# afiaka87/clip-guided-diffusion

Hardware: AMD Instinct MI355X
Metric: diffusion steps/sec (UNet+CLIP+grad) at 256x256 cutn=16 (higher is better)
Workload: dtype bf16x3 (split-bf16 MFMA, fp32 accumulate, fp32 storage); 1 GPU; BASELINE configs[1]: 256x256 class-cond UNet (554M), respace 250, cutn 16, batch 1/GPU, CLIP ViT-B/32, cgs 1000 tv 150 range 50, randomize_class, p_sample; global_batch=1, world_size_checked=1, collectives=none (single process)

## Files before the change

### clip-guided-diffusion_amd/csrc/vit.hip

```cpp
#include <memory>

#include "../../include/cgd_mi355x.h"
#include "net.h"

void ClipBlock::add_params(NetBase& net, const std::string& prefix, int width, int nheads) {
  pre = prefix;
  W = width;
  heads = nheads;
  net.add_param(pre + ".ln_1.weight", W);
  net.add_param(pre + ".ln_1.bias", W);
  net.add_param(pre + ".attn.in_proj_weight", (int64_t)3 * W * W);
  net.add_param(pre + ".attn.in_proj_bias", 3 * W);
  net.add_param(pre + ".attn.out_proj.weight", (int64_t)W * W);
  net.add_param(pre + ".attn.out_proj.bias", W);
  net.add_param(pre + ".ln_2.weight", W);
  net.add_param(pre + ".ln_2.bias", W);
  net.add_param(pre + ".mlp.c_fc.weight", (int64_t)4 * W * W);
  net.add_param(pre + ".mlp.c_fc.bias", 4 * W);
  net.add_param(pre + ".mlp.c_proj.weight", (int64_t)4 * W * W);
  net.add_param(pre + ".mlp.c_proj.bias", W);
}

void ClipBlock::lookup(NetBase& net) {
  ln1g = net.P(pre + ".ln_1.weight"); ln1b = net.P(pre + ".ln_1.bias");
  inw = net.P(pre + ".attn.in_proj_weight"); inb = net.P(pre + ".attn.in_proj_bias");
  ow = net.P(pre + ".attn.out_proj.weight"); ob = net.P(pre + ".attn.out_proj.bias");
  ln2g = net.P(pre + ".ln_2.weight"); ln2b = net.P(pre + ".ln_2.bias");
  fcw = net.P(pre + ".mlp.c_fc.weight"); fcb = net.P(pre + ".mlp.c_fc.bias");
  pjw = net.P(pre + ".mlp.c_proj.weight"); pjb = net.P(pre + ".mlp.c_proj.bias");
}

int clip_block_fwd(NetBase& net, const ClipBlock& b, ClipActs& t, const float* x, float* xo, int N, int T, bool causal, hipStream_t s) {
  cgd_ctx* ctx = net.ctx;
  const int W = b.W;
  const long rows = (long)N * T;
  CGD_TRY(net.ensure(t.st1, rows * 2)); CGD_TRY(net.ensure(t.st2, rows * 2));
  CGD_TRY(net.ensure(t.y, rows * W)); CGD_TRY(net.ensure(t.qkv, rows * 3 * W)); CGD_TRY(net.ensure(t.a, rows * W));
  CGD_TRY(net.ensure(t.x1, rows * W)); CGD_TRY(net.ensure(t.y2, rows * W)); CGD_TRY(net.ensure(t.u, rows * 4 * W));
  CGD_TRY(net.ensure(t.ga, rows * 4 * W));
  CGD_TRY(cgd_launch_ln_fwd(ctx, x, W, t.y.p, W, (int)rows, W, b.ln1g, b.ln1b, 1e-5f, t.st1.p, s));
  CGD_TRY(cgd_launch_gemm(ctx, lin(t.y.p, W, b.inw, W, t.qkv.p, 3 * W, b.inb, nullptr, 0, rows, 3 * W), s));
  const AttnShape sh{N, b.heads, T, W / b.heads, W, 0, causal ? 1 : 0};
  CGD_TRY(net.attn_fwd(t.att, sh, t.qkv.p, 3 * W, t.a.p, W, s));
  CGD_TRY(cgd_launch_gemm(ctx, lin(t.a.p, W, b.ow, W, t.x1.p, W, b.ob, x, W, rows, W, 1), s));
  CGD_TRY(cgd_launch_ln_fwd(ctx, t.x1.p, W, t.y2.p, W, (int)rows, W, b.ln2g, b.ln2b, 1e-5f, t.st2.p, s));
  {
    GemmParams fc = lin(t.y2.p, W, b.fcw, W, t.u.p, 4 * W, b.fcb, nullptr, 0, rows, 4 * W);
    if (cgd_gemm_fuses_act(ctx, fc)) {
      fc.act_out = t.ga.p; fc.ld_act = 4 * W; fc.act = b.act;
      CGD_TRY(cgd_launch_gemm(ctx, fc, s));
    } else {
      CGD_TRY(cgd_launch_gemm(ctx, fc, s));
      CGD_TRY(cgd_launch_act_fwd(ctx, t.u.p, t.ga.p, rows * 4 * W, b.act, s));
    }
  }
  return cgd_launch_gemm(ctx, lin(t.ga.p, 4 * W, b.pjw, 4 * W, xo, W, b.pjb, t.x1.p, W, rows, W, 1), s);
}

namespace {

struct Layer : ClipBlock {
  float *inwT = 0, *owT = 0, *fcwT = 0, *pjwT = 0;
  ClipActs f;
  DevBuf xo;
  DevBuf dga, du, dy2, dx1, da, dqkv, dy, dx;
};

struct ViT : NetBase {
  cgd_vit_config cfg;
  int g = 0, L = 0, W = 0, PP = 0;
  std::vector<Layer> layers;
  float *convw = 0, *convwT = 0, *cls = 0, *pos = 0, *lnpre_g = 0, *lnpre_b = 0, *lnpost_g = 0, *lnpost_b = 0, *proj = 0, *projT = 0;
  int N = 0, layout = 0;
  bool have_fwd = false;
  int fwd_prec = 0;
  DevBuf cols, pe, tok, st_pre, x0, st_post, clsn, dclsn, dxl, dtok, dcols;

  int build();
  int finalize(hipStream_t s);
  int forward(const float* img, int layout, int N, float* emb, hipStream_t s);
  int dgrad(const float* demb, float* dimg, hipStream_t s);
};

int ViT::build() {
  g = cfg.resolution / cfg.patch;
  L = g * g + 1;
  W = cfg.width;
  PP = 3 * cfg.patch * cfg.patch;
  if (cfg.resolution % cfg.patch) CGD_FAIL(ctx, "vit: resolution must be a multiple of the patch size");
  if (W % cfg.heads || (W / cfg.heads) % 4) CGD_FAIL(ctx, "vit: bad head configuration");
  add_param("conv1.weight", (int64_t)W * PP);
  add_param("class_embedding", W);
  add_param("positional_embedding", (int64_t)L * W);
  add_param("ln_pre.weight", W);
  add_param("ln_pre.bias", W);
  layers.resize(cfg.layers);
  for (int l = 0; l < cfg.layers; ++l) layers[l].add_params(*this, "transformer.resblocks." + std::to_string(l), W, cfg.heads);
  add_param("ln_post.weight", W);
  add_param("ln_post.bias", W);
  add_param("proj", (int64_t)W * cfg.out_dim);
  return 0;
}

int ViT::finalize(hipStream_t s) {
  CGD_TRY(check_all_set());
  convw = P("conv1.weight"); cls = P("class_embedding"); pos = P("positional_embedding");
  lnpre_g = P("ln_pre.weight"); lnpre_b = P("ln_pre.bias");
  lnpost_g = P("ln_post.weight"); lnpost_b = P("ln_post.bias");
  proj = P("proj");
  CGD_TRY(transpose_weight(convw, &convwT, W, PP, s));
  CGD_TRY(transpose_weight(proj, &projT, W, cfg.out_dim, s));
  for (Layer& l : layers) {
    l.lookup(*this);
    CGD_TRY(transpose_weight(l.inw, &l.inwT, 3 * W, W, s));
    CGD_TRY(transpose_weight(l.ow, &l.owT, W, W, s));
    CGD_TRY(transpose_weight(l.fcw, &l.fcwT, 4 * W, W, s));
    CGD_TRY(transpose_weight(l.pjw, &l.pjwT, W, 4 * W, s));
  }
  CGD_HIP(ctx, hipStreamSynchronize(s));
  finalized = true;
  have_fwd = false;
  return 0;
}

int ViT::forward(const float* img, int lay, int Nn, float* emb, hipStream_t s) {
  if (!finalized) CGD_FAIL(ctx, "vit: finalize() has not been called after the last set_param");
  N = Nn; layout = lay; have_fwd = false;
  fwd_prec = ctx->precision;
  const long rows = (long)N * L;
  const float* colp = img;
  if (layout == 0) {
    CGD_TRY(ensure(cols, (size_t)N * g * g * PP));
    CGD_TRY(cgd_launch_patchify(ctx, img, cols.p, N, cfg.resolution, cfg.patch, s));
    colp = cols.p;
  }
  CGD_TRY(ensure(pe, (size_t)N * g * g * W));
  CGD_TRY(ensure(tok, rows * W));
  CGD_TRY(ensure(x0, rows * W));
  CGD_TRY(ensure(st_pre, rows * 2));
  CGD_TRY(cgd_launch_gemm(ctx, lin(colp, PP, convw, PP, pe.p, W, nullptr, nullptr, 0, (long)N * g * g, W), s));
  CGD_TRY(cgd_launch_vit_tokens(ctx, pe.p, cls, pos, tok.p, N, L, W, s));
  CGD_TRY(cgd_launch_ln_fwd(ctx, tok.p, W, x0.p, W, (int)rows, W, lnpre_g, lnpre_b, 1e-5f, st_pre.p, s));
  const float* x = x0.p;
  for (Layer& l : layers) {
    CGD_TRY(ensure(l.xo, rows * W));
    CGD_TRY(clip_block_fwd(*this, l, l.f, x, l.xo.p, N, L, false, s));
    x = l.xo.p;
  }
  CGD_TRY(ensure(st_post, (size_t)N * 2));
  CGD_TRY(ensure(clsn, (size_t)N * W));
  CGD_TRY(cgd_launch_ln_fwd(ctx, x, L * W, clsn.p, W, N, W, lnpost_g, lnpost_b, 1e-5f, st_post.p, s));
  CGD_TRY(cgd_launch_gemm(ctx, lin(clsn.p, W, projT, W, emb, cfg.out_dim, nullptr, nullptr, 0, N, cfg.out_dim), s));
  have_fwd = true;
  return 0;
}

int ViT::dgrad(const float* demb, float* dimg, hipStream_t s) {
  if (!finalized) CGD_FAIL(ctx, "vit: finalize() has not been called after the last set_param");
  if (!have_fwd) CGD_FAIL(ctx, "vit: dgrad() needs a preceding forward()");
  if (fwd_prec != ctx->precision) CGD_FAIL(ctx, "vit: dgrad() under another precision mode than its forward()");
  const long rows = (long)N * L;
  const int H = cfg.heads, d = W / H;
  CGD_TRY(ensure(dclsn, (size_t)N * W));
  CGD_TRY(ensure(dxl, rows * W));
  CGD_TRY(cgd_launch_gemm(ctx, lin(demb, cfg.out_dim, proj, cfg.out_dim, dclsn.p, W, nullptr, nullptr, 0, N, W), s));
  CGD_TRY(cgd_launch_fill(ctx, dxl.p, rows * W, 0.f, s));
  const float* xlast = layers.empty() ? x0.p : layers.back().xo.p;
  CGD_TRY(cgd_launch_ln_bwd(ctx, xlast, L * W, dclsn.p, W, dxl.p, L * W, nullptr, 0, N, W, lnpost_g, st_post.p, s));
  const float* dcur = dxl.p;
  for (int li = (int)layers.size() - 1; li >= 0; --li) {
    Layer& l = layers[li];
    const float* xin = li == 0 ? x0.p : layers[li - 1].xo.p;
    CGD_TRY(ensure(l.dga, rows * 4 * W)); CGD_TRY(ensure(l.du, rows * 4 * W)); CGD_TRY(ensure(l.dy2, rows * W));
    CGD_TRY(ensure(l.dx1, rows * W)); CGD_TRY(ensure(l.da, rows * W)); CGD_TRY(ensure(l.dqkv, rows * 3 * W));
    CGD_TRY(ensure(l.dy, rows * W)); CGD_TRY(ensure(l.dx, rows * W));
    {
      GemmParams pj = lin(dcur, W, l.pjwT, W, l.dga.p, 4 * W, nullptr, nullptr, 0, rows, 4 * W);
      if (cgd_gemm_fuses_act(ctx, pj)) {
        pj.C = l.du.p;
        pj.act_in = l.f.u.p; pj.ld_act = 4 * W; pj.act = l.act;
        CGD_TRY(cgd_launch_gemm(ctx, pj, s));
      } else {
        CGD_TRY(cgd_launch_gemm(ctx, pj, s));
        CGD_TRY(cgd_launch_act_bwd(ctx, l.f.u.p, l.dga.p, l.du.p, rows * 4 * W, l.act, s));
      }
    }
    CGD_TRY(cgd_launch_gemm(ctx, lin(l.du.p, 4 * W, l.fcwT, 4 * W, l.dy2.p, W, nullptr, nullptr, 0, rows, W, 1), s));
    CGD_TRY(cgd_launch_ln_bwd(ctx, l.f.x1.p, W, l.dy2.p, W, l.dx1.p, W, dcur, W, (int)rows, W, l.ln2g, l.f.st2.p, s));
    CGD_TRY(cgd_launch_gemm(ctx, lin(l.dx1.p, W, l.owT, W, l.da.p, W, nullptr, nullptr, 0, rows, W), s));
    CGD_TRY(attn_bwd(l.f.att, AttnShape{N, H, L, d, W, 0, 0}, l.f.qkv.p, 3 * W, l.da.p, W, l.dqkv.p, 3 * W, s));
    CGD_TRY(cgd_launch_gemm(ctx, lin(l.dqkv.p, 3 * W, l.inwT, 3 * W, l.dy.p, W, nullptr, nullptr, 0, rows, W, 1), s));
    CGD_TRY(cgd_launch_ln_bwd(ctx, xin, W, l.dy.p, W, l.dx.p, W, l.dx1.p, W, (int)rows, W, l.ln1g, l.f.st1.p, s));
    dcur = l.dx.p;
  }
  CGD_TRY(ensure(dtok, rows * W));
  CGD_TRY(cgd_launch_ln_bwd(ctx, tok.p, W, dcur, W, dtok.p, W, nullptr, 0, (int)rows, W, lnpre_g, st_pre.p, s));
  float* dc = dimg;
  if (layout == 0) {
    CGD_TRY(ensure(dcols, (size_t)N * g * g * PP));
    dc = dcols.p;
  }
  GemmParams one = lin(dtok.p, W, convwT, W, dc, PP, nullptr, nullptr, 0, rows, PP);
  one.no_split = 1;
  if (cgd_gemm_fuses_act(ctx, one)) {
    one.skip_group = L;
    CGD_TRY(cgd_launch_gemm(ctx, one, s));
  } else {
    GemmParams p;
    p.A = dtok.p + W; p.lda = W; p.B = convwT; p.ldb = W; p.C = dc; p.ldc = PP; p.M = g * g; p.N = PP; p.K = W;
    p.nbatch = N; p.bdiv = 1; p.sA1 = (long)L * W; p.sC1 = (long)g * g * PP;
    CGD_TRY(cgd_launch_gemm(ctx, p, s));
  }
  if (layout == 0) CGD_TRY(cgd_launch_unpatchify(ctx, dcols.p, dimg, N, cfg.resolution, cfg.patch, s));
  return 0;
}

}

struct cgd_vit {
  ViT net;
};

extern "C" {
int cgd_vit_create(cgd_ctx* ctx, const cgd_vit_config* cfg, cgd_vit** out) { return net_create(ctx, out, cfg); }
int cgd_vit_manifest(const cgd_vit_config* cfg, void (*cb)(const char*, int64_t, void*), void* user) { return net_manifest<ViT>(cb, user, cfg); }
void cgd_vit_destroy(cgd_vit* v) { net_destroy(v); }
int cgd_vit_num_params(cgd_vit* v) { return net_num_params(v); }
int cgd_vit_param_info(cgd_vit* v, int i, char* buf, int len, int64_t* numel) { return net_param_info(v, i, buf, len, numel); }
int cgd_vit_set_param(cgd_vit* v, const char* name, const float* data, int64_t numel) { return net_set_param(v, name, data, numel); }
int cgd_vit_finalize(cgd_vit* v) { return net_finalize(v); }
int cgd_vit_set_activation(cgd_vit* v, int act) {
  if (!v) return -3;
  v->net.have_fwd = false;
  return clip_set_activation(v->net.ctx, v->net.layers, act);
}
int cgd_vit_forward(cgd_vit* v, const float* img, int layout, int N, float* emb, void* stream) {
  return net_pass(v, stream, [&](hipStream_t s) { return v->net.forward(img, layout, N, emb, s); });
}
int cgd_vit_dgrad(cgd_vit* v, const float* d_emb, float* d_img, void* stream) {
  return net_pass(v, stream, [&](hipStream_t s) { return v->net.dgrad(d_emb, d_img, s); });
}
}
```

Baseline: 59.30 diffusion steps/sec.

## Compute only CLS-token rows after attention in the final ViT block

The last CLIP transformer block now runs the out-projection, ln_2, MLP and residual only for the class token of each image, because the pooled embedding reads nothing else. Its backward pass writes the class-token gradients into a preallocated zeroed buffer with a row stride, so attention backward still sees full-shaped inputs; that buffer is zero-filled once and reused across calls. Separately, the out-projection dgrad GEMM in the other layers turns off split-K when the half-precision GEMM path already has enough tiles to fill the CUs. This adds a special code path for the final layer and relies on the non-class rows of the cached buffer staying zero.

After: 59.49 diffusion steps/sec, median of 6. No clear change (+0.3%).

```diff
diff --git a/clip-guided-diffusion_amd/csrc/vit.hip b/clip-guided-diffusion_amd/csrc/vit.hip
--- a/clip-guided-diffusion_amd/csrc/vit.hip
+++ b/clip-guided-diffusion_amd/csrc/vit.hip
@@ -64,6 +64,9 @@
   ClipActs f;
   DevBuf xo;
   DevBuf dga, du, dy2, dx1, da, dqkv, dy, dx;
+  DevBuf zr;
+  const float* zr_filled = nullptr;
+  long zr_rows = 0;
 };
 
 struct ViT : NetBase {
@@ -73,6 +76,7 @@
   float *convw = 0, *convwT = 0, *cls = 0, *pos = 0, *lnpre_g = 0, *lnpre_b = 0, *lnpost_g = 0, *lnpost_b = 0, *proj = 0, *projT = 0;
   int N = 0, layout = 0;
   bool have_fwd = false;
+  bool tail_fwd = false;
   int fwd_prec = 0;
   DevBuf cols, pe, tok, st_pre, x0, st_post, clsn, dclsn, dxl, dtok, dcols;
 
@@ -80,6 +84,8 @@
   int finalize(hipStream_t s);
   int forward(const float* img, int layout, int N, float* emb, hipStream_t s);
   int dgrad(const float* demb, float* dimg, hipStream_t s);
+  int tail_block_fwd(Layer& l, const float* x, hipStream_t s);
+  int tail_block_bwd(Layer& l, const float* xin, const float* dxo, hipStream_t s);
 };
 
 int ViT::build() {
@@ -123,6 +129,61 @@
   return 0;
 }
 
+int ViT::tail_block_fwd(Layer& l, const float* x, hipStream_t s) {
+  ClipActs& t = l.f;
+  const long rows = (long)N * L;
+  const int ldc = L * W;
+  CGD_TRY(ensure(t.st1, rows * 2)); CGD_TRY(ensure(t.st2, (size_t)N * 2));
+  CGD_TRY(ensure(t.y, rows * W)); CGD_TRY(ensure(t.qkv, rows * 3 * W)); CGD_TRY(ensure(t.a, rows * W));
+  CGD_TRY(ensure(t.x1, (size_t)N * W)); CGD_TRY(ensure(t.y2, (size_t)N * W)); CGD_TRY(ensure(t.u, (size_t)N * 4 * W));
+  CGD_TRY(ensure(t.ga, (size_t)N * 4 * W)); CGD_TRY(ensure(l.xo, (size_t)N * W));
+  CGD_TRY(cgd_launch_ln_fwd(ctx, x, W, t.y.p, W, (int)rows, W, l.ln1g, l.ln1b, 1e-5f, t.st1.p, s));
+  CGD_TRY(cgd_launch_gemm(ctx, lin(t.y.p, W, l.inw, W, t.qkv.p, 3 * W, l.inb, nullptr, 0, rows, 3 * W), s));
+  const AttnShape sh{N, l.heads, L, W / l.heads, W, 0, 0};
+  CGD_TRY(attn_fwd(t.att, sh, t.qkv.p, 3 * W, t.a.p, W, s));
+  CGD_TRY(cgd_launch_gemm(ctx, lin(t.a.p, ldc, l.ow, W, t.x1.p, W, l.ob, x, ldc, N, W), s));
+  CGD_TRY(cgd_launch_ln_fwd(ctx, t.x1.p, W, t.y2.p, W, N, W, l.ln2g, l.ln2b, 1e-5f, t.st2.p, s));
+  GemmParams fc = lin(t.y2.p, W, l.fcw, W, t.u.p, 4 * W, l.fcb, nullptr, 0, N, 4 * W);
+  if (cgd_gemm_fuses_act(ctx, fc)) {
+    fc.act_out = t.ga.p; fc.ld_act = 4 * W; fc.act = l.act;
+    CGD_TRY(cgd_launch_gemm(ctx, fc, s));
+  } else {
+    CGD_TRY(cgd_launch_gemm(ctx, fc, s));
+    CGD_TRY(cgd_launch_act_fwd(ctx, t.u.p, t.ga.p, (long)N * 4 * W, l.act, s));
+  }
+  return cgd_launch_gemm(ctx, lin(t.ga.p, 4 * W, l.pjw, 4 * W, l.xo.p, W, l.pjb, t.x1.p, W, N, W), s);
+}
+
+int ViT::tail_block_bwd(Layer& l, const float* xin, const float* dxo, hipStream_t s) {
+  const long rows = (long)N * L;
+  const int H = cfg.heads, d = W / H, ldc = L * W;
+  CGD_TRY(ensure(l.dga, (size_t)N * 4 * W)); CGD_TRY(ensure(l.du, (size_t)N * 4 * W)); CGD_TRY(ensure(l.dy2, (size_t)N * W));
+  CGD_TRY(ensure(l.zr, 2 * rows * W)); CGD_TRY(ensure(l.dqkv, rows * 3 * W));
+  CGD_TRY(ensure(l.dy, rows * W)); CGD_TRY(ensure(l.dx, rows * W));
+  float* const dx1 = l.zr.p;
+  float* const da = l.zr.p + rows * W;
+  if (l.zr_filled != l.zr.p || l.zr_rows != rows) {
+    CGD_TRY(cgd_launch_fill(ctx, l.zr.p, 2 * rows * W, 0.f, s));
+    l.zr_filled = l.zr.p;
+    l.zr_rows = rows;
+  }
+  GemmParams pj = lin(dxo, W, l.pjwT, W, l.dga.p, 4 * W, nullptr, nullptr, 0, N, 4 * W);
+  if (cgd_gemm_fuses_act(ctx, pj)) {
+    pj.C = l.du.p;
+    pj.act_in = l.f.u.p; pj.ld_act = 4 * W; pj.act = l.act;
+    CGD_TRY(cgd_launch_gemm(ctx, pj, s));
+  } else {
+    CGD_TRY(cgd_launch_gemm(ctx, pj, s));
+    CGD_TRY(cgd_launch_act_bwd(ctx, l.f.u.p, l.dga.p, l.du.p, (long)N * 4 * W, l.act, s));
+  }
+  CGD_TRY(cgd_launch_gemm(ctx, lin(l.du.p, 4 * W, l.fcwT, 4 * W, l.dy2.p, W, nullptr, nullptr, 0, N, W), s));
+  CGD_TRY(cgd_launch_ln_bwd(ctx, l.f.x1.p, W, l.dy2.p, W, dx1, ldc, dxo, W, N, W, l.ln2g, l.f.st2.p, s));
+  CGD_TRY(cgd_launch_gemm(ctx, lin(dx1, ldc, l.owT, W, da, ldc, nullptr, nullptr, 0, N, W), s));
+  CGD_TRY(attn_bwd(l.f.att, AttnShape{N, H, L, d, W, 0, 0}, l.f.qkv.p, 3 * W, da, W, l.dqkv.p, 3 * W, s));
+  CGD_TRY(cgd_launch_gemm(ctx, lin(l.dqkv.p, 3 * W, l.inwT, 3 * W, l.dy.p, W, nullptr, nullptr, 0, rows, W, 1), s));
+  return cgd_launch_ln_bwd(ctx, xin, W, l.dy.p, W, l.dx.p, W, dx1, W, (int)rows, W, l.ln1g, l.f.st1.p, s);
+}
+
 int ViT::forward(const float* img, int lay, int Nn, float* emb, hipStream_t s) {
   if (!finalized) CGD_FAIL(ctx, "vit: finalize() has not been called after the last set_param");
   N = Nn; layout = lay; have_fwd = false;
@@ -142,14 +203,22 @@
   CGD_TRY(cgd_launch_vit_tokens(ctx, pe.p, cls, pos, tok.p, N, L, W, s));
   CGD_TRY(cgd_launch_ln_fwd(ctx, tok.p, W, x0.p, W, (int)rows, W, lnpre_g, lnpre_b, 1e-5f, st_pre.p, s));
   const float* x = x0.p;
-  for (Layer& l : layers) {
+  tail_fwd = !layers.empty();
+  for (size_t li = 0; li + 1 < layers.size(); ++li) {
+    Layer& l = layers[li];
     CGD_TRY(ensure(l.xo, rows * W));
     CGD_TRY(clip_block_fwd(*this, l, l.f, x, l.xo.p, N, L, false, s));
     x = l.xo.p;
   }
+  int ldx = L * W;
+  if (tail_fwd) {
+    CGD_TRY(tail_block_fwd(layers.back(), x, s));
+    x = layers.back().xo.p;
+    ldx = W;
+  }
   CGD_TRY(ensure(st_post, (size_t)N * 2));
   CGD_TRY(ensure(clsn, (size_t)N * W));
-  CGD_TRY(cgd_launch_ln_fwd(ctx, x, L * W, clsn.p, W, N, W, lnpost_g, lnpost_b, 1e-5f, st_post.p, s));
+  CGD_TRY(cgd_launch_ln_fwd(ctx, x, ldx, clsn.p, W, N, W, lnpost_g, lnpost_b, 1e-5f, st_post.p, s));
   CGD_TRY(cgd_launch_gemm(ctx, lin(clsn.p, W, projT, W, emb, cfg.out_dim, nullptr, nullptr, 0, N, cfg.out_dim), s));
   have_fwd = true;
   return 0;
@@ -162,13 +231,23 @@
   const long rows = (long)N * L;
   const int H = cfg.heads, d = W / H;
   CGD_TRY(ensure(dclsn, (size_t)N * W));
-  CGD_TRY(ensure(dxl, rows * W));
   CGD_TRY(cgd_launch_gemm(ctx, lin(demb, cfg.out_dim, proj, cfg.out_dim, dclsn.p, W, nullptr, nullptr, 0, N, W), s));
-  CGD_TRY(cgd_launch_fill(ctx, dxl.p, rows * W, 0.f, s));
-  const float* xlast = layers.empty() ? x0.p : layers.back().xo.p;
-  CGD_TRY(cgd_launch_ln_bwd(ctx, xlast, L * W, dclsn.p, W, dxl.p, L * W, nullptr, 0, N, W, lnpost_g, st_post.p, s));
-  const float* dcur = dxl.p;
-  for (int li = (int)layers.size() - 1; li >= 0; --li) {
+  const float* dcur = nullptr;
+  int nfull = (int)layers.size();
+  if (tail_fwd) {
+    Layer& l = layers.back();
+    --nfull;
+    CGD_TRY(ensure(dxl, (size_t)N * W));
+    CGD_TRY(cgd_launch_ln_bwd(ctx, l.xo.p, W, dclsn.p, W, dxl.p, W, nullptr, 0, N, W, lnpost_g, st_post.p, s));
+    CGD_TRY(tail_block_bwd(l, nfull == 0 ? x0.p : layers[nfull - 1].xo.p, dxl.p, s));
+    dcur = l.dx.p;
+  } else {
+    CGD_TRY(ensure(dxl, rows * W));
+    CGD_TRY(cgd_launch_fill(ctx, dxl.p, rows * W, 0.f, s));
+    CGD_TRY(cgd_launch_ln_bwd(ctx, x0.p, L * W, dclsn.p, W, dxl.p, L * W, nullptr, 0, N, W, lnpost_g, st_post.p, s));
+    dcur = dxl.p;
+  }
+  for (int li = nfull - 1; li >= 0; --li) {
     Layer& l = layers[li];
     const float* xin = li == 0 ? x0.p : layers[li - 1].xo.p;
     CGD_TRY(ensure(l.dga, rows * 4 * W)); CGD_TRY(ensure(l.du, rows * 4 * W)); CGD_TRY(ensure(l.dy2, rows * W));
@@ -187,7 +266,11 @@
     }
     CGD_TRY(cgd_launch_gemm(ctx, lin(l.du.p, 4 * W, l.fcwT, 4 * W, l.dy2.p, W, nullptr, nullptr, 0, rows, W, 1), s));
     CGD_TRY(cgd_launch_ln_bwd(ctx, l.f.x1.p, W, l.dy2.p, W, l.dx1.p, W, dcur, W, (int)rows, W, l.ln2g, l.f.st2.p, s));
-    CGD_TRY(cgd_launch_gemm(ctx, lin(l.dx1.p, W, l.owT, W, l.da.p, W, nullptr, nullptr, 0, rows, W), s));
+    {
+      GemmParams ow = lin(l.dx1.p, W, l.owT, W, l.da.p, W, nullptr, nullptr, 0, rows, W);
+      ow.no_split = cgd_hgemm_supported(ctx, ow) && 4L * cgd_hgemm_tiles(ctx, ow) > ctx->num_cu;
+      CGD_TRY(cgd_launch_gemm(ctx, ow, s));
+    }
     CGD_TRY(attn_bwd(l.f.att, AttnShape{N, H, L, d, W, 0, 0}, l.f.qkv.p, 3 * W, l.da.p, W, l.dqkv.p, 3 * W, s));
     CGD_TRY(cgd_launch_gemm(ctx, lin(l.dqkv.p, 3 * W, l.inwT, 3 * W, l.dy.p, W, nullptr, nullptr, 0, rows, W, 1), s));
     CGD_TRY(cgd_launch_ln_bwd(ctx, xin, W, l.dy.p, W, l.dx.p, W, l.dx1.p, W, (int)rows, W, l.ln1g, l.f.st1.p, s));
```
